# salemon/quattro-transformer-ilqr

Measured on AMD Instinct MI355X. Metric: iLQR iterations/sec (batch x horizon steps/s), quadrotor N=50 batch=4096, higher is better.
Workload: dtype f32; 1 GPU; quadrotor n_x=12 n_u=4 N=50, pure iLQR iteration = simulate (nominal rollout + cost) + linearisation and Riccati sweep (one fused launch) + 6-alpha line search/commit (BASELINE configs[2]; configs[3] when n_gpus=8); batch_per_gpu=4096, global_batch=4096, horizon=50, n_x=12, n_u=4, integrator=euler, parallelism=dp1 (independent trajectory shards)

## Files before the change

quattro-transformer-ilqr_amd/csrc/rollout_quad_body.h:

```cpp
#pragma once
#include <type_traits>

#include "models_device.h"

namespace {

constexpr int NX = 12, NU = 4, CS = 16;

#define QT_QP(a, b, c, d) ((a) | ((b) << 2) | ((c) << 4) | ((d) << 6))
template <int CTRL>
__device__ __forceinline__ float quad_perm(float v) {
  return __builtin_bit_cast(float, __builtin_amdgcn_update_dpp(0, __builtin_bit_cast(int, v), CTRL, 0xf, 0xf, true));
}
template <int I>
__device__ __forceinline__ float quad_bcast(float v) {
  return quad_perm<QT_QP(I, I, I, I)>(v);
}
__device__ __forceinline__ double quad_sum(double v) {
  v += __shfl_xor(v, 1);
  v += __shfl_xor(v, 2);
  return v;
}

struct LaneConst {
  bool is0, is1;
  int a, j;
  float qw[4], qfw[4], xr[4];
  float rj;
  float tc[4];
  float gy, gz, inv_mass, dt;
  __device__ __forceinline__ float sel(float v0, float v1, float v2) const { return is0 ? v0 : (is1 ? v1 : v2); }
};

__device__ __forceinline__ LaneConst lane_const(const quattro_model_params& p, int j) {
  LaneConst L;
  L.j = j;
  L.a = j == 3 ? 0 : j;
  L.is0 = L.a == 0;
  L.is1 = L.a == 1;
  const float live = j == 3 ? 0.0f : 1.0f;
#pragma unroll
  for (int g = 0; g < 4; ++g) {
    L.qw[g] = live * L.sel(p.q[3 * g], p.q[3 * g + 1], p.q[3 * g + 2]);
    L.qfw[g] = live * L.sel(p.qf[3 * g], p.qf[3 * g + 1], p.qf[3 * g + 2]);
    L.xr[g] = L.sel(p.x_ref[3 * g], p.x_ref[3 * g + 1], p.x_ref[3 * g + 2]);
  }
  L.rj = p.r[j];
  const float Ix = p.phys[1], Iy = p.phys[2], Iz = p.phys[3], arm = p.phys[4], kyaw = p.phys[6];
  const float s0 = L.sel(-1.0f, 1.0f, 1.0f), s1 = L.sel(1.0f, 1.0f, -1.0f), s2 = L.sel(1.0f, -1.0f, 1.0f),
              s3 = L.sel(-1.0f, -1.0f, -1.0f);
  const float gain = L.sel(arm / Ix, arm / Iy, kyaw / Iz);
  L.tc[0] = s0 * gain; L.tc[1] = s1 * gain; L.tc[2] = s2 * gain; L.tc[3] = s3 * gain;
  L.gy = L.sel((Iy - Iz) / Ix, (Iz - Ix) / Iy, (Ix - Iy) / Iz);
  L.gz = L.sel(0.0f, 0.0f, -p.phys[5]);
  L.inv_mass = 1.0f / p.phys[0];
  L.dt = p.dt;
  return L;
}

__device__ __forceinline__ LaneConst lane_const_plant(const PlantSpec& plant, const float* __restrict__ plant_phys, size_t bb,
                                                      float dt, int j) {
  float ph[7];
#pragma unroll
  for (int i = 0; i < 7; ++i) ph[i] = plant.phys[i];
  if (plant_phys != nullptr) {
#pragma unroll
    for (int i = 0; i < 7; ++i) ph[i] = plant_phys[bb * 8 + i];
  }
  const float mass = ph[0], Ix = ph[1], Iy = ph[2], Iz = ph[3], arm = ph[4], grav = ph[5], kyaw = ph[6];
  LaneConst L{};
  L.j = j;
  L.a = j == 3 ? 0 : j;
  L.is0 = L.a == 0;
  L.is1 = L.a == 1;
  const float s0 = L.sel(-1.0f, 1.0f, 1.0f), s1 = L.sel(1.0f, 1.0f, -1.0f), s2 = L.sel(1.0f, -1.0f, 1.0f),
              s3 = L.sel(-1.0f, -1.0f, -1.0f);
  const float gain = L.sel(arm / Ix, arm / Iy, kyaw / Iz);
  L.tc[0] = s0 * gain; L.tc[1] = s1 * gain; L.tc[2] = s2 * gain; L.tc[3] = s3 * gain;
  L.gy = L.sel((Iy - Iz) / Ix, (Iz - Ix) / Iy, (Ix - Iy) / Iz);
  L.gz = L.sel(0.0f, 0.0f, -grav);
  L.inv_mass = 1.0f / mass;
  L.dt = dt;
  return L;
}

__device__ __forceinline__ LaneConst lane_const_phys(const quattro_model_params& p, const float* __restrict__ model_phys, size_t bb,
                                                     int j) {
  LaneConst L = lane_const(p, j);
  float ph[7];
#pragma unroll
  for (int i = 0; i < 7; ++i) ph[i] = model_phys[bb * 8 + i];
  const float mass = ph[0], Ix = ph[1], Iy = ph[2], Iz = ph[3], arm = ph[4], grav = ph[5], kyaw = ph[6];
  const float s0 = L.sel(-1.0f, 1.0f, 1.0f), s1 = L.sel(1.0f, 1.0f, -1.0f), s2 = L.sel(1.0f, -1.0f, 1.0f),
              s3 = L.sel(-1.0f, -1.0f, -1.0f);
  const float gain = L.sel(arm / Ix, arm / Iy, kyaw / Iz);
  L.tc[0] = s0 * gain; L.tc[1] = s1 * gain; L.tc[2] = s2 * gain; L.tc[3] = s3 * gain;
  L.gy = L.sel((Iy - Iz) / Ix, (Iz - Ix) / Iy, (Ix - Iy) / Iz);
  L.gz = L.sel(0.0f, 0.0f, -grav);
  L.inv_mass = 1.0f / mass;
  return L;
}

template <bool PHYS>
__device__ __forceinline__ LaneConst lane_const_of(const quattro_model_params& p, const float* __restrict__ model_phys, size_t bb,
                                                   int j) {
  if constexpr (PHYS) return lane_const_phys(p, model_phys, bb, j);
  else return lane_const(p, j);
}

struct QuadU {
  float u0, u1, u2, u3;
  __device__ __forceinline__ explicit QuadU(float uo)
      : u0(quad_bcast<0>(uo)), u1(quad_bcast<1>(uo)), u2(quad_bcast<2>(uo)), u3(quad_bcast<3>(uo)) {}
};

struct TrigBase {
  float a, s, c;
};
__device__ __forceinline__ void stage_sincos(const TrigBase& b, float x, float* s, float* c) {
  const float d = x - b.a;
  if (__builtin_expect(__any(!(fabsf(d) <= 0.25f)), 0)) {
    qt_sincos(x, s, c);
    return;
  }
  const float z = d * d;
  const float sd = d * fmaf(z, fmaf(z, fmaf(z, -1.9841270e-4f, 8.3333333e-3f), -1.6666667e-1f), 1.0f);
  const float cd = fmaf(z, fmaf(z, fmaf(z, -1.3888889e-3f, 4.1666667e-2f), -0.5f), 1.0f);
  *s = fmaf(b.s, cd, b.c * sd);
  *c = fmaf(b.c, cd, -(b.s * sd));
}

template <bool STAGE>
__device__ __forceinline__ void quad_rate(const LaneConst& L, const float* xo, const QuadU& U, float* xd, TrigBase& tb) {
  const float u0 = U.u0, u1 = U.u1, u2 = U.u2, u3 = U.u3;
  const float tm = (u0 + u1 + u2 + u3) * L.inv_mass;
  const float tau = fmaf(L.tc[3], u3, fmaf(L.tc[2], u2, fmaf(L.tc[1], u1, L.tc[0] * u0)));
  float so, co;
  if constexpr (STAGE) {
    stage_sincos(tb, xo[2], &so, &co);
  } else {
    qt_sincos_chain(xo[2], &so, &co);
    tb.a = xo[2]; tb.s = so; tb.c = co;
  }
  const float sph = quad_bcast<0>(so), cph = quad_bcast<0>(co), sth = quad_bcast<1>(so), cth = quad_bcast<1>(co),
              sps = quad_bcast<2>(so), cps = quad_bcast<2>(co);
  const float y = __builtin_amdgcn_rcpf(cth);
  const float sec = fmaf(fmaf(-cth, y, 1.0f), y, y);
  const float tth = sth * sec;
  const float wp = quad_bcast<0>(xo[3]), wq = quad_bcast<1>(xo[3]), wr = quad_bcast<2>(xo[3]);
  xd[0] = xo[1];
  const float ca = L.sel(sps, cps, 0.0f), cb = L.sel(cps * sth, -(sps * sth), cth);
  xd[1] = fmaf(tm, fmaf(ca, sph, cb * cph), L.gz);
  const float mix = fmaf(wq, sph, wr * cph);
  xd[2] = L.sel(fmaf(mix, tth, wp), fmaf(wq, cph, -(wr * sph)), mix * sec);
  xd[3] = fmaf(L.gy, L.sel(wq * wr, wp * wr, wp * wq), tau);
}

template <bool RK4>
__device__ __forceinline__ void quad_step(const LaneConst& L, const float* xo, const QuadU& uo, float* xn) {
  TrigBase tb;
  if constexpr (!RK4) {
    float k1[4];
    quad_rate<false>(L, xo, uo, k1, tb);
#pragma unroll
    for (int g = 0; g < 4; ++g) xn[g] = fmaf(L.dt, k1[g], xo[g]);
  } else {
    rk4_step<4>(L.dt, xo, xn, [&](int s, const float* xs, float* k) __attribute__((always_inline)) {
      if (s == 0) quad_rate<false>(L, xs, uo, k, tb);
      else quad_rate<true>(L, xs, uo, k, tb);
    });
  }
}

__device__ __forceinline__ float lane_stage_cost(const quattro_model_params& p, const LaneConst& L, const float* xo,
                                                 float uo, unsigned long long counted) {
  float c = 0.0f;
#pragma unroll
  for (int g = 0; g < 4; ++g) {
    const float d = xo[g] - L.xr[g];
    c = fmaf(L.qw[g] * d, d, c);
  }
  c = fmaf(L.rj * uo, uo, c);
  if (p.barrier_alpha != 0.0f) {
    const float ib = 1.0f / p.barrier_beta;
    const unsigned long long big = __builtin_amdgcn_ballot_w64(p.barrier_beta * uo > 20.0f);
    const unsigned long long tiny = __builtin_amdgcn_ballot_w64(fabsf(p.barrier_alpha) * 4.25e-18f * ib * ib < c * 2.9e-8f);
    if ((counted & ~(big & tiny)) != 0ull) {
      const float sp = qt_softplus(-uo, p.barrier_beta);
      c = fmaf(p.barrier_alpha, sp * sp, c);
    }
  }
  return c;
}

__device__ __forceinline__ float lane_final_cost(const LaneConst& L, const float* xo) {
  float c = 0.0f;
#pragma unroll
  for (int g = 0; g < 4; ++g) {
    const float d = xo[g] - L.xr[g];
    c = fmaf(L.qfw[g] * d, d, c);
  }
  return c;
}

struct NomSrc {
  __amdgpu_buffer_rsrc_t rx, ru, rK, rk;
  int vx, vu, vK;
  __device__ __forceinline__ NomSrc(const LaneConst& L, const float* x_nom, const float* u_nom, const float* K, const float* k,
                                    int N, int wb, int li, int nwt) {
    const size_t w = (size_t)wb;
    rx = __builtin_amdgcn_make_buffer_rsrc(const_cast<float*>(x_nom) + w * (N + 1) * NX, 0, nwt * (N + 1) * NX * 4, 0x00020000);
    ru = __builtin_amdgcn_make_buffer_rsrc(const_cast<float*>(u_nom) + w * N * NU, 0, nwt * N * NU * 4, 0x00020000);
    rK = __builtin_amdgcn_make_buffer_rsrc(const_cast<float*>(K) + w * N * NU * NX, 0, nwt * N * NU * NX * 4, 0x00020000);
    rk = __builtin_amdgcn_make_buffer_rsrc(const_cast<float*>(k) + w * N * NU, 0, nwt * N * NU * 4, 0x00020000);
    vx = 4 * (li * (N + 1) * NX + L.a);
    vu = 4 * (li * N * NU + L.j);
    vK = 4 * NX * (li * N * NU + L.j);
  }
};

struct NomLane {
  float x[4], u, k;
  float4 K[3];
  __device__ __forceinline__ void load(const NomSrc& s, int t) {
#pragma unroll
    for (int g = 0; g < 4; ++g) x[g] = __int_as_float(__builtin_amdgcn_raw_buffer_load_b32(s.rx, s.vx + 12 * g, t * (NX * 4), 0));
    u = __int_as_float(__builtin_amdgcn_raw_buffer_load_b32(s.ru, s.vu, t * (NU * 4), 0));
    k = __int_as_float(__builtin_amdgcn_raw_buffer_load_b32(s.rk, s.vu, t * (NU * 4), 0));
#pragma unroll
    for (int i = 0; i < 3; ++i) {
      const auto q = __builtin_amdgcn_raw_buffer_load_b128(s.rK, s.vK + 16 * i, t * (NU * NX * 4), 0);
      K[i] = make_float4(__int_as_float(q[0]), __int_as_float(q[1]), __int_as_float(q[2]), __int_as_float(q[3]));
    }
  }
  __device__ __forceinline__ void load_track(const NomSrc& s, int t) {
#pragma unroll
    for (int g = 0; g < 4; ++g) x[g] = __int_as_float(__builtin_amdgcn_raw_buffer_load_b32(s.rx, s.vx + 12 * g, t * (NX * 4), 0));
    u = __int_as_float(__builtin_amdgcn_raw_buffer_load_b32(s.ru, s.vu, t * (NU * 4), 0));
#pragma unroll
    for (int i = 0; i < 3; ++i) {
      const auto q = __builtin_amdgcn_raw_buffer_load_b128(s.rK, s.vK + 16 * i, t * (NU * NX * 4), 0);
      K[i] = make_float4(__int_as_float(q[0]), __int_as_float(q[1]), __int_as_float(q[2]), __int_as_float(q[3]));
    }
  }
};

struct NoRefSrc {
  static constexpr bool ON = false;
  __device__ __forceinline__ NoRefSrc() {}
  __device__ __forceinline__ NoRefSrc(const LaneConst&, const RefRows&, int, int, int) {}
};
struct RefSrc {
  static constexpr bool ON = true;
  __amdgpu_buffer_rsrc_t r;
  int v;
  RefRows rr;
  __device__ __forceinline__ RefSrc(const LaneConst& L, const RefRows& rr_, int wb, int li, int nwt) : rr(rr_) {
    r = __builtin_amdgcn_make_buffer_rsrc(const_cast<float*>(rr_.rows) + (size_t)wb * rr_.R * NX, 0, nwt * rr_.R * NX * 4, 0x00020000);
    v = 4 * (li * rr_.R * NX + L.a);
  }
};
struct RefLane {
  float xr[4];
  __device__ __forceinline__ void load(const RefSrc& s, int t) {
    const int row = qt_ref_row(s.rr, t);
#pragma unroll
    for (int g = 0; g < 4; ++g) xr[g] = __int_as_float(__builtin_amdgcn_raw_buffer_load_b32(s.r, s.v + 12 * g, row * (NX * 4), 0));
  }
  __device__ __forceinline__ void load(const NoRefSrc&, int) {}
};
template <class RefS>
__device__ __forceinline__ LaneConst with_ref(const LaneConst& L, const RefLane& rl) {
  if constexpr (RefS::ON) {
    LaneConst Lt = L;
#pragma unroll
    for (int g = 0; g < 4; ++g) Lt.xr[g] = rl.xr[g];
    return Lt;
  } else {
    return L;
  }
}

__device__ __forceinline__ float4 gather_quarter(const LaneConst& L, const QuadU& U, const float* xn) {
  const float t0 = L.sel(xn[0], xn[1], xn[2]);
  const float t1 = quad_perm<QT_QP(1, 2, 0, 3)>(L.sel(xn[3], xn[0], xn[1]));
  const float t2 = quad_perm<QT_QP(2, 0, 1, 3)>(L.sel(xn[2], xn[3], xn[0]));
  const float t3 = L.sel(xn[1], xn[2], xn[3]);
  const bool l3 = L.j == 3;
  return make_float4(l3 ? U.u0 : t0, l3 ? U.u1 : t1, l3 ? U.u2 : t2, l3 ? U.u3 : t3);
}

struct NoStore {
  __device__ __forceinline__ void operator()(const LaneConst&, int, const QuadU&, const float*) const {}
};
struct ArrayStore {
  float* base;
  int stride;
  bool en;
  __device__ __forceinline__ ArrayStore(const LaneConst& L, float* xo, float* uo, bool en_)
      : base(L.j < 3 ? xo + NX + 4 * L.j : uo), stride(L.j < 3 ? NX : NU), en(en_) {}
  __device__ __forceinline__ void operator()(const LaneConst& L, int t, const QuadU& U, const float* xnext) const {
    const float4 v = gather_quarter(L, U, xnext);
    if (en) *reinterpret_cast<float4*>(base + (size_t)t * stride) = v;
  }
};
struct ScratchStore {
  float* s;
  bool en, l3;
  __device__ __forceinline__ ScratchStore(const LaneConst& L, float* rec, bool en_) : s(rec + 4 * L.j), en(en_), l3(L.j == 3) {}
  __device__ __forceinline__ void operator()(const LaneConst&, int t, const QuadU& U, const float* xnext) const {
    const float4 v = make_float4(l3 ? U.u0 : xnext[0], l3 ? U.u1 : xnext[1], l3 ? U.u2 : xnext[2], l3 ? U.u3 : xnext[3]);
    if (en) *reinterpret_cast<float4*>(s + (size_t)t * CS) = v;
  }
};

__device__ __forceinline__ float gain_dot(const float4* K, const float* dx, float acc) {
#define QT_FD(k, d, l) "v_fmac_f32_dpp %0, " d ", " k " quad_perm:[" l "," l "," l "," l "] row_mask:0xf bank_mask:0xf bound_ctrl:1\n\t"
  asm volatile("s_nop 1\n\t"
               QT_FD("%5", "%1", "0") QT_FD("%6", "%1", "1") QT_FD("%7", "%1", "2")
               QT_FD("%8", "%2", "0") QT_FD("%9", "%2", "1") QT_FD("%10", "%2", "2")
               QT_FD("%11", "%3", "0") QT_FD("%12", "%3", "1") QT_FD("%13", "%3", "2")
               QT_FD("%14", "%4", "0") QT_FD("%15", "%4", "1") QT_FD("%16", "%4", "2")
               : "+v"(acc)
               : "v"(dx[0]), "v"(dx[1]), "v"(dx[2]), "v"(dx[3]), "v"(K[0].x), "v"(K[0].y), "v"(K[0].z), "v"(K[0].w),
                 "v"(K[1].x), "v"(K[1].y), "v"(K[1].z), "v"(K[1].w), "v"(K[2].x), "v"(K[2].y), "v"(K[2].z), "v"(K[2].w));
#undef QT_FD
  return acc;
}

__device__ __forceinline__ void quad_track_body(const LaneConst& L, const bool rk4, const bool feedback, const NomSrc& nom,
                                                float* xh, const int steps, const float* __restrict__ dist,
                                                const size_t dist_stride, const bool live, float* __restrict__ xrows,
                                                float* __restrict__ urows) {
#pragma clang fp contract(off)
  for (int j = 0; j < steps; ++j) {
    NomLane nb;
    nb.load_track(nom, j);
    float ua = nb.u;
    if (feedback) {
      float dx[4];
#pragma unroll
      for (int g = 0; g < 4; ++g) dx[g] = xh[g] - nb.x[g];
      ua = gain_dot(nb.K, dx, ua);
    }
    const QuadU U(ua);
    float xn[4];
    if (rk4) quad_step<true>(L, xh, U, xn);
    else quad_step<false>(L, xh, U, xn);
    if (dist != nullptr) {
#pragma unroll
      for (int g = 0; g < 4; ++g) xn[g] += dist[(size_t)j * dist_stride + 3 * g];
    }
    if (live) {
      urows[(size_t)j * NU] = ua;
      if (L.j < 3) {
#pragma unroll
        for (int g = 0; g < 4; ++g) xrows[(size_t)(j + 1) * NX + 3 * g] = xn[g];
      }
    }
#pragma unroll
    for (int g = 0; g < 4; ++g) xh[g] = xn[g];
  }
}

template <bool RK4, int PF, bool PRIO, class Store, class RefS = NoRefSrc>
__device__ __forceinline__ double quad_rollout_closed(const quattro_model_params& p, const LaneConst& L,
                                                      const NomSrc& src, float alpha, int N, bool counted, Store store,
                                                      const RefS& ref = RefS()) {
  const unsigned long long counted_mask = __builtin_amdgcn_ballot_w64(counted);
  NomLane nb[PF];
#pragma unroll
  for (int d = 0; d < PF; ++d) nb[d].load(src, d < N ? d : N - 1);
  RefLane rl[PF], rlN;
#pragma unroll
  for (int d = 0; d < PF; ++d) rl[d].load(ref, d < N ? d : N - 1);
  rlN.load(ref, N);
  float xh[4];
#pragma unroll
  for (int g = 0; g < 4; ++g) xh[g] = nb[0].x[g];
  double J = 0.0;
  auto step = [&](const NomLane& b, const RefLane& rt, int t) __attribute__((always_inline)) {
    if constexpr (PRIO) __builtin_amdgcn_s_setprio(1);
    float dx[4];
#pragma unroll
    for (int g = 0; g < 4; ++g) dx[g] = xh[g] - b.x[g];
    const float du = gain_dot(b.K, dx, b.k);
    const float uh = fmaf(alpha, du, b.u);
    if constexpr (!PRIO) J += (double)lane_stage_cost(p, with_ref<RefS>(L, rt), xh, uh, counted_mask);
    float xnext[4];
    const QuadU U(uh);
    quad_step<RK4>(L, xh, U, xnext);
    if constexpr (PRIO) {
      __builtin_amdgcn_s_setprio(0);
      J += (double)lane_stage_cost(p, with_ref<RefS>(L, rt), xh, uh, counted_mask);
    }
    store(L, t, U, xnext);
#pragma unroll
    for (int g = 0; g < 4; ++g) xh[g] = xnext[g];
  };
  int t = 0;
  for (; t + PF <= N; t += PF) {
#pragma unroll
    for (int d = 0; d < PF; ++d) {
      step(nb[d], rl[d], t + d);
      nb[d].load(src, t + d + PF < N ? t + d + PF : N - 1);
      rl[d].load(ref, t + d + PF < N ? t + d + PF : N - 1);
    }
  }
#pragma unroll
  for (int d = 0; d < PF - 1; ++d)
    if (t + d < N) step(nb[d], rl[d], t + d);
  J += (double)lane_final_cost(with_ref<RefS>(L, rlN), xh);
  return J;
}

template <bool RK4, bool PHYS = false, bool REF = false>
__device__ __forceinline__ void simulate_quad_body(const quattro_model_params& p, const float* __restrict__ x0,
                                                   const float* __restrict__ u, int N, float* __restrict__ x,
                                                   double* __restrict__ cost, const int gid, const bool live,
                                                   const float* __restrict__ model_phys = nullptr, const RefRows& rr = RefRows{}) {
  using RefS = std::conditional_t<REF, RefSrc, NoRefSrc>;
  const int b = gid >> 2;
  const size_t bb = live ? b : 0;
  const LaneConst L = lane_const_of<PHYS>(p, model_phys, bb, gid & 3);
  const float* ub = u + bb * N * NU + L.j;
  float* xo = x + bb * (N + 1) * NX + L.a;
  float xh[4];
#pragma unroll
  for (int g = 0; g < 4; ++g) xh[g] = x0[bb * NX + 3 * g + L.a];
  const bool writer = live && L.j < 3;
  const int bw = __builtin_amdgcn_readfirstlane(b);
  const __amdgpu_buffer_rsrc_t rsx =
      __builtin_amdgcn_make_buffer_rsrc(x + (size_t)bw * (N + 1) * NX, 0, 16 * (N + 1) * NX * 4, 0x00020000);
  const int vox = writer ? 4 * ((b - bw) * (N + 1) * NX + L.a) : -1;
  if (writer) {
#pragma unroll
    for (int g = 0; g < 4; ++g) xo[3 * g] = xh[g];
  }
  const RefS ref(L, rr, bw, live ? b - bw : 0, 16);
  RefLane r0, r1, rN;
  r0.load(ref, 0);
  r1.load(ref, N > 1 ? 1 : 0);
  rN.load(ref, N);
  double J = 0.0;
  const unsigned long long live_mask = __builtin_amdgcn_ballot_w64(live);
  float u0 = ub[0], u1 = ub[(size_t)(N > 1 ? 1 : 0) * NU];
  auto step = [&](float ut, const RefLane& rt, int t) __attribute__((always_inline)) {
    J += (double)lane_stage_cost(p, with_ref<RefS>(L, rt), xh, ut, live_mask);
    float xn[4];
    const QuadU U(ut);
    quad_step<RK4>(L, xh, U, xn);
#pragma unroll
    for (int g = 0; g < 4; ++g)
      __builtin_amdgcn_raw_buffer_store_b32(__float_as_int(xn[g]), rsx, vox, (t + 1) * (NX * 4) + 12 * g, 0);
#pragma unroll
    for (int g = 0; g < 4; ++g) xh[g] = xn[g];
  };
  asm volatile("" : "+v"(u0), "+v"(u1));
  if constexpr (REF) {
#pragma unroll
    for (int g = 0; g < 4; ++g) asm volatile("" : "+v"(r0.xr[g]), "+v"(r1.xr[g]), "+v"(rN.xr[g]));
  }
  __builtin_amdgcn_s_waitcnt(0x0f70);
  int t = 0;
  for (; t + 1 < N; t += 2) {
    step(u0, r0, t);
    u0 = ub[(size_t)(t + 2 < N ? t + 2 : N - 1) * NU];
    r0.load(ref, t + 2 < N ? t + 2 : N - 1);
    step(u1, r1, t + 1);
    u1 = ub[(size_t)(t + 3 < N ? t + 3 : N - 1) * NU];
    r1.load(ref, t + 3 < N ? t + 3 : N - 1);
  }
  if (t < N) step(u0, r0, t);
  J += (double)lane_final_cost(with_ref<RefS>(L, rN), xh);
  J = quad_sum(J);
  if (live && L.j == 0 && cost != nullptr) cost[b] = J;
}

template <bool RK4, int PF, bool PRIO, bool PHYS = false, bool REF = false>
__device__ __forceinline__ void linesearch_quad_body(const quattro_model_params& p, float* x_nom, float* u_nom,
                                                     const float* __restrict__ K, const float* __restrict__ k,
                                                     const AlphaList& al, int n_alpha, int B, int N, double tol,
                                                     double* cost, int32_t* __restrict__ alpha_idx, int32_t* active,
                                                     int32_t* iters, float* __restrict__ scratch, const int gid,
                                                     const bool force, const float* __restrict__ model_phys = nullptr,
                                                     const RefRows& rr = RefRows{}) {
  const int b = gid >> 5, ai = (gid >> 2) & 7, l32 = gid & 31;
  const bool live = (b < B) && (force || active == nullptr || active[b < B ? b : 0] != 0);
  if (!__any(live)) return;
  const bool mine = live && ai < n_alpha;
  const size_t bb = live ? b : 0;
  const int aa = mine ? ai : 0;
  const LaneConst L = lane_const_of<PHYS>(p, model_phys, bb, gid & 3);
  float* xn = x_nom + bb * (N + 1) * NX;
  float* un = u_nom + bb * N * NU;
  const int wb = __builtin_amdgcn_readfirstlane(b);
  const NomSrc nom(L, x_nom, u_nom, K, k, N, wb, live ? b - wb : 0, 2);
  float* sc = scratch + (bb * 8) * (size_t)N * CS;
  float alpha = al.a[0];
#pragma unroll
  for (int i = 1; i < QUATTRO_MAX_ALPHAS; ++i) alpha = (aa == i) ? al.a[i] : alpha;
  const double J0 = live ? cost[bb] : 0.0;
  using RefS = std::conditional_t<REF, RefSrc, NoRefSrc>;
  double J = quad_rollout_closed<RK4, PF, PRIO>(p, L, nom, alpha, N, mine, ScratchStore(L, sc + (size_t)aa * N * CS, mine),
                                                RefS(L, rr, wb, live ? b - wb : 0, 2));
  J = quad_sum(J);
  const bool ok = mine && (J <= J0);
  const unsigned long long bal = __ballot(ok);
  const int lane = threadIdx.x & 63;
  const unsigned grp = (unsigned)((bal >> (lane & 32)) & 0x11111111ull);
  const int first = grp ? ((__ffs((int)grp) - 1) >> 2) : -1;
  if (live && first >= 0) {
    __builtin_amdgcn_fence(__ATOMIC_RELEASE, "workgroup");
    asm volatile("s_waitcnt vmcnt(0)" ::: "memory");
    __builtin_amdgcn_fence(__ATOMIC_ACQUIRE, "workgroup");
    const float* src = sc + (size_t)first * N * CS;
    const int e = l32 & 15, half = l32 >> 4;
    const bool isx = e < 12;
    const int slot = isx ? 4 * (e % 3) + e / 3 : e;
    float* dst = isx ? xn + NX + e : un + (e - 12);
    const int dstride = isx ? NX : NU;
    constexpr int COPY_U = 13;
    for (int t0 = half; t0 < N; t0 += 2 * COPY_U) {
      float v[COPY_U];
#pragma unroll
      for (int q = 0; q < COPY_U; ++q) {
        const int t = t0 + 2 * q;
        v[q] = src[(size_t)(t < N ? t : t0) * CS + slot];
      }
#pragma unroll
      for (int q = 0; q < COPY_U; ++q) {
        const int t = t0 + 2 * q;
        if (t < N) dst[(size_t)t * dstride] = v[q];
      }
    }
    if (ai == first && L.j == 0) {
      cost[b] = J;
      if (active != nullptr && fabs(J0 - J) < tol) active[b] = 0;
    }
  }
  if (live && l32 == 0) {
    if (alpha_idx != nullptr) alpha_idx[b] = first;
    if (iters != nullptr) iters[b] += 1;
    if (first < 0 && active != nullptr) active[b] = 0;
  }
}

}
```

Before: 1.975 billion steps/s.

## Fuse control broadcast into DPP ops, buffer-load controls, widen commit copy unroll

```diff
diff --git a/quattro-transformer-ilqr_amd/csrc/rollout_quad_body.h b/quattro-transformer-ilqr_amd/csrc/rollout_quad_body.h
--- a/quattro-transformer-ilqr_amd/csrc/rollout_quad_body.h
+++ b/quattro-transformer-ilqr_amd/csrc/rollout_quad_body.h
@@ -32,6 +32,10 @@
   __device__ __forceinline__ float sel(float v0, float v1, float v2) const { return is0 ? v0 : (is1 ? v1 : v2); }
 };
 
+__device__ __forceinline__ void pin_torque_row(LaneConst& L) {
+  asm("" : "+v"(L.tc[0]), "+v"(L.tc[1]), "+v"(L.tc[2]), "+v"(L.tc[3]));
+}
+
 __device__ __forceinline__ LaneConst lane_const(const quattro_model_params& p, int j) {
   LaneConst L;
   L.j = j;
@@ -51,6 +55,7 @@
               s3 = L.sel(-1.0f, -1.0f, -1.0f);
   const float gain = L.sel(arm / Ix, arm / Iy, kyaw / Iz);
   L.tc[0] = s0 * gain; L.tc[1] = s1 * gain; L.tc[2] = s2 * gain; L.tc[3] = s3 * gain;
+  pin_torque_row(L);
   L.gy = L.sel((Iy - Iz) / Ix, (Iz - Ix) / Iy, (Ix - Iy) / Iz);
   L.gz = L.sel(0.0f, 0.0f, -p.phys[5]);
   L.inv_mass = 1.0f / p.phys[0];
@@ -77,6 +82,7 @@
               s3 = L.sel(-1.0f, -1.0f, -1.0f);
   const float gain = L.sel(arm / Ix, arm / Iy, kyaw / Iz);
   L.tc[0] = s0 * gain; L.tc[1] = s1 * gain; L.tc[2] = s2 * gain; L.tc[3] = s3 * gain;
+  pin_torque_row(L);
   L.gy = L.sel((Iy - Iz) / Ix, (Iz - Ix) / Iy, (Ix - Iy) / Iz);
   L.gz = L.sel(0.0f, 0.0f, -grav);
   L.inv_mass = 1.0f / mass;
@@ -95,6 +101,7 @@
               s3 = L.sel(-1.0f, -1.0f, -1.0f);
   const float gain = L.sel(arm / Ix, arm / Iy, kyaw / Iz);
   L.tc[0] = s0 * gain; L.tc[1] = s1 * gain; L.tc[2] = s2 * gain; L.tc[3] = s3 * gain;
+  pin_torque_row(L);
   L.gy = L.sel((Iy - Iz) / Ix, (Iz - Ix) / Iy, (Ix - Iy) / Iz);
   L.gz = L.sel(0.0f, 0.0f, -grav);
   L.inv_mass = 1.0f / mass;
@@ -109,9 +116,39 @@
 }
 
 struct QuadU {
-  float u0, u1, u2, u3;
-  __device__ __forceinline__ explicit QuadU(float uo)
-      : u0(quad_bcast<0>(uo)), u1(quad_bcast<1>(uo)), u2(quad_bcast<2>(uo)), u3(quad_bcast<3>(uo)) {}
+  float own;
+  bool all;
+  float c[4];
+  __device__ __forceinline__ explicit QuadU(float uo, bool want_all = false) : own(uo), all(want_all) {
+    if (all) { c[0] = quad_bcast<0>(uo); c[1] = quad_bcast<1>(uo); c[2] = quad_bcast<2>(uo); c[3] = quad_bcast<3>(uo); }
+  }
+};
+
+struct QuadDrive {
+  float tm, tau;
+  __device__ __forceinline__ QuadDrive(const LaneConst& L, const QuadU& U) {
+    if (U.all) {
+      tm = (U.c[0] + U.c[1] + U.c[2] + U.c[3]) * L.inv_mass;
+      tau = fmaf(L.tc[3], U.c[3], fmaf(L.tc[2], U.c[2], fmaf(L.tc[1], U.c[1], L.tc[0] * U.c[0])));
+      return;
+    }
+    float s, t;
+#define QT_DP(l) " quad_perm:[" l "," l "," l "," l "] row_mask:0xf bank_mask:0xf bound_ctrl:1\n\t"
+    asm volatile("s_nop 1\n\t"
+                 "v_mov_b32_dpp %0, %2" QT_DP("0")
+                 "v_mul_f32_dpp %1, %2, %3" QT_DP("0")
+                 "v_add_f32_dpp %0, %2, %0" QT_DP("1")
+                 "v_fmac_f32_dpp %1, %2, %4" QT_DP("1")
+                 "v_add_f32_dpp %0, %2, %0" QT_DP("2")
+                 "v_fmac_f32_dpp %1, %2, %5" QT_DP("2")
+                 "v_add_f32_dpp %0, %2, %0" QT_DP("3")
+                 "v_fmac_f32_dpp %1, %2, %6" QT_DP("3")
+                 : "=&v"(s), "=&v"(t)
+                 : "v"(U.own), "v"(L.tc[0]), "v"(L.tc[1]), "v"(L.tc[2]), "v"(L.tc[3]));
+#undef QT_DP
+    tm = s * L.inv_mass;
+    tau = t;
+  }
 };
 
 struct TrigBase {
@@ -131,10 +168,8 @@
 }
 
 template <bool STAGE>
-__device__ __forceinline__ void quad_rate(const LaneConst& L, const float* xo, const QuadU& U, float* xd, TrigBase& tb) {
-  const float u0 = U.u0, u1 = U.u1, u2 = U.u2, u3 = U.u3;
-  const float tm = (u0 + u1 + u2 + u3) * L.inv_mass;
-  const float tau = fmaf(L.tc[3], u3, fmaf(L.tc[2], u2, fmaf(L.tc[1], u1, L.tc[0] * u0)));
+__device__ __forceinline__ void quad_rate(const LaneConst& L, const float* xo, const QuadDrive& D, float* xd, TrigBase& tb) {
+  const float tm = D.tm, tau = D.tau;
   float so, co;
   if constexpr (STAGE) {
     stage_sincos(tb, xo[2], &so, &co);
@@ -153,23 +188,31 @@
   xd[1] = fmaf(tm, fmaf(ca, sph, cb * cph), L.gz);
   const float mix = fmaf(wq, sph, wr * cph);
   xd[2] = L.sel(fmaf(mix, tth, wp), fmaf(wq, cph, -(wr * sph)), mix * sec);
-  xd[3] = fmaf(L.gy, L.sel(wq * wr, wp * wr, wp * wq), tau);
+  xd[3] = fmaf(L.gy, quad_perm<QT_QP(1, 0, 0, 1)>(xo[3]) * quad_perm<QT_QP(2, 2, 1, 2)>(xo[3]), tau);
 }
 
 template <bool RK4>
 __device__ __forceinline__ void quad_step(const LaneConst& L, const float* xo, const QuadU& uo, float* xn) {
+  const QuadDrive D(L, uo);
   TrigBase tb;
   if constexpr (!RK4) {
     float k1[4];
-    quad_rate<false>(L, xo, uo, k1, tb);
+    quad_rate<false>(L, xo, D, k1, tb);
 #pragma unroll
     for (int g = 0; g < 4; ++g) xn[g] = fmaf(L.dt, k1[g], xo[g]);
   } else {
     rk4_step<4>(L.dt, xo, xn, [&](int s, const float* xs, float* k) __attribute__((always_inline)) {
-      if (s == 0) quad_rate<false>(L, xs, uo, k, tb);
-      else quad_rate<true>(L, xs, uo, k, tb);
+      if (s == 0) quad_rate<false>(L, xs, D, k, tb);
+      else quad_rate<true>(L, xs, D, k, tb);
     });
   }
+}
+
+__device__ __forceinline__ unsigned long long barrier_lanes(const quattro_model_params& p, bool counted) {
+  const bool on = (__float_as_uint(p.barrier_alpha) << 1) != 0u;
+  unsigned long long m = on ? __builtin_amdgcn_ballot_w64(counted) : 0ull;
+  asm volatile("" : "+s"(m));
+  return m;
 }
 
 __device__ __forceinline__ float lane_stage_cost(const quattro_model_params& p, const LaneConst& L, const float* xo,
@@ -181,14 +224,12 @@
     c = fmaf(L.qw[g] * d, d, c);
   }
   c = fmaf(L.rj * uo, uo, c);
-  if (p.barrier_alpha != 0.0f) {
-    const float ib = 1.0f / p.barrier_beta;
-    const unsigned long long big = __builtin_amdgcn_ballot_w64(p.barrier_beta * uo > 20.0f);
-    const unsigned long long tiny = __builtin_amdgcn_ballot_w64(fabsf(p.barrier_alpha) * 4.25e-18f * ib * ib < c * 2.9e-8f);
-    if ((counted & ~(big & tiny)) != 0ull) {
-      const float sp = qt_softplus(-uo, p.barrier_beta);
-      c = fmaf(p.barrier_alpha, sp * sp, c);
-    }
+  const float ib = 1.0f / p.barrier_beta;
+  const unsigned long long big = __builtin_amdgcn_ballot_w64(p.barrier_beta * uo > 20.0f);
+  const unsigned long long tiny = __builtin_amdgcn_ballot_w64(fabsf(p.barrier_alpha) * 4.25e-18f * ib * ib < c * 2.9e-8f);
+  if ((counted & ~(big & tiny)) != 0ull) {
+    const float sp = qt_softplus(-uo, p.barrier_beta);
+    c = fmaf(p.barrier_alpha, sp * sp, c);
   }
   return c;
 }
@@ -287,13 +328,15 @@
   const float t2 = quad_perm<QT_QP(2, 0, 1, 3)>(L.sel(xn[2], xn[3], xn[0]));
   const float t3 = L.sel(xn[1], xn[2], xn[3]);
   const bool l3 = L.j == 3;
-  return make_float4(l3 ? U.u0 : t0, l3 ? U.u1 : t1, l3 ? U.u2 : t2, l3 ? U.u3 : t3);
+  return make_float4(l3 ? U.c[0] : t0, l3 ? U.c[1] : t1, l3 ? U.c[2] : t2, l3 ? U.c[3] : t3);
 }
 
 struct NoStore {
+  static constexpr bool ALL_U = false;
   __device__ __forceinline__ void operator()(const LaneConst&, int, const QuadU&, const float*) const {}
 };
 struct ArrayStore {
+  static constexpr bool ALL_U = true;
   float* base;
   int stride;
   bool en;
@@ -305,11 +348,12 @@
   }
 };
 struct ScratchStore {
+  static constexpr bool ALL_U = true;
   float* s;
   bool en, l3;
   __device__ __forceinline__ ScratchStore(const LaneConst& L, float* rec, bool en_) : s(rec + 4 * L.j), en(en_), l3(L.j == 3) {}
   __device__ __forceinline__ void operator()(const LaneConst&, int t, const QuadU& U, const float* xnext) const {
-    const float4 v = make_float4(l3 ? U.u0 : xnext[0], l3 ? U.u1 : xnext[1], l3 ? U.u2 : xnext[2], l3 ? U.u3 : xnext[3]);
+    const float4 v = make_float4(l3 ? U.c[0] : xnext[0], l3 ? U.c[1] : xnext[1], l3 ? U.c[2] : xnext[2], l3 ? U.c[3] : xnext[3]);
     if (en) *reinterpret_cast<float4*>(s + (size_t)t * CS) = v;
   }
 };
@@ -367,7 +411,7 @@
 __device__ __forceinline__ double quad_rollout_closed(const quattro_model_params& p, const LaneConst& L,
                                                       const NomSrc& src, float alpha, int N, bool counted, Store store,
                                                       const RefS& ref = RefS()) {
-  const unsigned long long counted_mask = __builtin_amdgcn_ballot_w64(counted);
+  const unsigned long long counted_mask = barrier_lanes(p, counted);
   NomLane nb[PF];
 #pragma unroll
   for (int d = 0; d < PF; ++d) nb[d].load(src, d < N ? d : N - 1);
@@ -388,7 +432,7 @@
     const float uh = fmaf(alpha, du, b.u);
     if constexpr (!PRIO) J += (double)lane_stage_cost(p, with_ref<RefS>(L, rt), xh, uh, counted_mask);
     float xnext[4];
-    const QuadU U(uh);
+    const QuadU U(uh, Store::ALL_U);
     quad_step<RK4>(L, xh, U, xnext);
     if constexpr (PRIO) {
       __builtin_amdgcn_s_setprio(0);
@@ -423,7 +467,6 @@
   const int b = gid >> 2;
   const size_t bb = live ? b : 0;
   const LaneConst L = lane_const_of<PHYS>(p, model_phys, bb, gid & 3);
-  const float* ub = u + bb * N * NU + L.j;
   float* xo = x + bb * (N + 1) * NX + L.a;
   float xh[4];
 #pragma unroll
@@ -432,7 +475,16 @@
   const int bw = __builtin_amdgcn_readfirstlane(b);
   const __amdgpu_buffer_rsrc_t rsx =
       __builtin_amdgcn_make_buffer_rsrc(x + (size_t)bw * (N + 1) * NX, 0, 16 * (N + 1) * NX * 4, 0x00020000);
-  const int vox = writer ? 4 * ((b - bw) * (N + 1) * NX + L.a) : -1;
+  const int vox = writer ? 4 * ((b - bw) * (N + 1) * NX + L.a) : 0x40000000;
+  int uflags = 0x00020000;
+  asm("" : "+s"(uflags));
+  const __amdgpu_buffer_rsrc_t rsu =
+      __builtin_amdgcn_make_buffer_rsrc(const_cast<float*>(u) + (size_t)bw * N * NU, 0, 16 * N * NU * 4, uflags);
+  const int vou = 4 * ((live ? b - bw : 0) * N * NU + L.j);
+  const int ou_last = (N - 1) * (NU * 4);
+  auto control = [&](int ofs) __attribute__((always_inline)) {
+    return __int_as_float(__builtin_amdgcn_raw_buffer_load_b32(rsu, vou, ofs < ou_last ? ofs : ou_last, 0));
+  };
   if (writer) {
 #pragma unroll
     for (int g = 0; g < 4; ++g) xo[3 * g] = xh[g];
@@ -443,8 +495,9 @@
   r1.load(ref, N > 1 ? 1 : 0);
   rN.load(ref, N);
   double J = 0.0;
-  const unsigned long long live_mask = __builtin_amdgcn_ballot_w64(live);
-  float u0 = ub[0], u1 = ub[(size_t)(N > 1 ? 1 : 0) * NU];
+  const unsigned long long live_mask = barrier_lanes(p, live);
+  float u0 = control(0), u1 = control(NU * 4);
+  int ou = 2 * (NU * 4);
   auto step = [&](float ut, const RefLane& rt, int t) __attribute__((always_inline)) {
     J += (double)lane_stage_cost(p, with_ref<RefS>(L, rt), xh, ut, live_mask);
     float xn[4];
@@ -452,7 +505,7 @@
     quad_step<RK4>(L, xh, U, xn);
 #pragma unroll
     for (int g = 0; g < 4; ++g)
-      __builtin_amdgcn_raw_buffer_store_b32(__float_as_int(xn[g]), rsx, vox, (t + 1) * (NX * 4) + 12 * g, 0);
+      __builtin_amdgcn_raw_buffer_store_b32(__float_as_int(xn[g]), rsx, vox + 12 * g, (t + 1) * (NX * 4), 0);
 #pragma unroll
     for (int g = 0; g < 4; ++g) xh[g] = xn[g];
   };
@@ -465,10 +518,12 @@
   int t = 0;
   for (; t + 1 < N; t += 2) {
     step(u0, r0, t);
-    u0 = ub[(size_t)(t + 2 < N ? t + 2 : N - 1) * NU];
+    u0 = control(ou);
+    ou += NU * 4;
     r0.load(ref, t + 2 < N ? t + 2 : N - 1);
     step(u1, r1, t + 1);
-    u1 = ub[(size_t)(t + 3 < N ? t + 3 : N - 1) * NU];
+    u1 = control(ou);
+    ou += NU * 4;
     r1.load(ref, t + 3 < N ? t + 3 : N - 1);
   }
   if (t < N) step(u0, r0, t);
@@ -520,7 +575,7 @@
     const int slot = isx ? 4 * (e % 3) + e / 3 : e;
     float* dst = isx ? xn + NX + e : un + (e - 12);
     const int dstride = isx ? NX : NU;
-    constexpr int COPY_U = 13;
+    constexpr int COPY_U = 25;
     for (int t0 = half; t0 < N; t0 += 2 * COPY_U) {
       float v[COPY_U];
 #pragma unroll
```

New measurement: 2.006 billion steps/s (median of 6 runs). +1.6%, better.
